# jdubkim/Self-play-on-Multi-Snakes-Environment

Hardware: AMD Instinct MI355X
Metric: env-steps/sec (agent·step) at 4 096×19×19×3-snake, 1/2/4/8 GPU + CPU ref (higher is better)
Workload: dtype u8

## Files before the change

### include/msnake.h

```cpp
#ifndef MSNAKE_H
#define MSNAKE_H

#include <stddef.h>
#include <stdint.h>

#ifdef __cplusplus
extern "C" {
#endif

#define MSNAKE_ABI_VERSION 3

#define MSNAKE_RULES_SNAKE_ENV 0
#define MSNAKE_RULES_NEW_WORLD 1
#define MSNAKE_RULES_ADVERSARIAL 2

#define MSNAKE_MAX_SNAKES 4
#define MSNAKE_MAX_FRUITS 32
#define MSNAKE_MAX_DIM 62

#define MSNAKE_OK 0
#define MSNAKE_E_ARG (-1)
#define MSNAKE_E_HIP (-2)
#define MSNAKE_E_HANDLE (-3)
#define MSNAKE_E_ALIGN (-4)
// ... 75 lines not shown
int msnake_set_state_all(msnake_handle h, const void* buf, size_t bytes);

typedef struct msnake_blob_info {
    int32_t version, num_envs, dim, n_snakes, n_fruits, rules;
    int64_t total_words;
} msnake_blob_info;
int msnake_state_blob_info(const void* buf, size_t bytes, msnake_blob_info* out);

int msnake_render(msnake_handle h, uint8_t* obs_dev, void* stream);

#define MSNAKE_POLICY_NONE 0
#define MSNAKE_POLICY_SAFE_GREEDY 1
#define MSNAKE_POLICY_HAMILTONIAN 2
int msnake_scripted_actions(msnake_handle h, int32_t policy, uint32_t snake_mask, int32_t* actions_dev,
                            int32_t action_stride, uint8_t* safe_dev, void* stream);

int msnake_space_actions(msnake_handle h, uint32_t snake_mask, int32_t* actions_dev, int32_t action_stride,
                         uint8_t* safe_dev, uint16_t* space_dev, void* stream);

int msnake_copy_envs(msnake_handle dst, msnake_handle src, const int32_t* src_index_dev, void* stream);

int msnake_render_cells(msnake_handle h, uint32_t view_mask, uint8_t* cells_dev, int32_t* snakes_dev, void* stream);

#define MSNAKE_LOCAL_MAX_RADIUS 31
#define MSNAKE_CELL_OUTSIDE 6
int msnake_render_local(msnake_handle h, int32_t radius, uint32_t snake_mask, int32_t oriented, uint8_t* windows_dev,
                        uint8_t* heading_dev, void* stream);

int msnake_get_stats(msnake_handle h, msnake_stats* out, int32_t reset);

const char* msnake_kernel_name(msnake_handle h);
int msnake_kernel_name_for_config(const msnake_config* cfg, char* out, size_t n);
int msnake_set_generic_kernels(int32_t on);
int64_t msnake_algorithmic_bytes_per_env_step(msnake_handle h);

#ifdef __cplusplus
}
#endif
#endif
```

### self-play-on-multi-snakes-environment_amd/_capi.py

```python
import ctypes
import os

_HERE = os.path.dirname(os.path.abspath(__file__))
LIB_PATH = os.environ.get("MSNAKE_LIB") or os.path.join(_HERE, "libmsnake.so")

RULES = {"snake_env": 0, "new_world": 1, "adversarial": 2}
RULE_NAMES = {v: k for k, v in RULES.items()}

SYMBOLS = [
    "msnake_abi_version", "msnake_last_error", "msnake_create", "msnake_destroy", "msnake_obs_shape",
    "msnake_reset", "msnake_reset_envs", "msnake_step", "msnake_step_tape", "msnake_rollout_tape", "msnake_get_state", "msnake_set_state",
    "msnake_get_state_all", "msnake_set_state_all", "msnake_state_blob_info",
    "msnake_render", "msnake_get_stats", "msnake_kernel_name", "msnake_algorithmic_bytes_per_env_step",
    "msnake_scripted_actions", "msnake_copy_envs", "msnake_kernel_name_for_config",
    "msnake_set_generic_kernels", "msnake_space_actions", "msnake_render_cells", "msnake_render_local",
]


class MsnakeConfig(ctypes.Structure):
    _fields_ = [("struct_size", ctypes.c_uint32), ("device", ctypes.c_int32), ("num_envs", ctypes.c_int32),
                ("dim", ctypes.c_int32), ("n_snakes", ctypes.c_int32), ("n_fruits", ctypes.c_int32),
                ("rules", ctypes.c_int32), ("max_steps", ctypes.c_int32), ("auto_reset", ctypes.c_int32),
                ("obs_scale", ctypes.c_int32), ("seed", ctypes.c_uint64), ("env_id_base", ctypes.c_uint64),
                ("envs_per_block", ctypes.c_int32), ("record_policy", ctypes.c_int32),
                ("obs_store_policy", ctypes.c_int32), ("tape_store_policy", ctypes.c_int32)]


ABI_VERSION = 3
CONFIG_SIZE_V2 = 56
RECORD_POLICY = {"auto": 0, "full": 1, "short": 2}
STORE_POLICY = {"auto": 0, "plain": 1, "stream": 2}
SCRIPTED_POLICY = {None: 0, "safe_greedy": 1, "hamiltonian": 2}
SPACE_POLICY = "space_greedy"


class MsnakeBlobInfo(ctypes.Structure):
    _fields_ = [("version", ctypes.c_int32), ("num_envs", ctypes.c_int32), ("dim", ctypes.c_int32),
                ("n_snakes", ctypes.c_int32), ("n_fruits", ctypes.c_int32), ("rules", ctypes.c_int32),
                ("total_words", ctypes.c_int64)]


class MsnakeStats(ctypes.Structure):
    _fields_ = [("episodes", ctypes.c_int64), ("ep_len_sum", ctypes.c_int64), ("ep_return_sum", ctypes.c_int64),
                ("env_steps", ctypes.c_int64), ("errors", ctypes.c_int64), ("reserved", ctypes.c_int64 * 3)]


_lib = None

# ... 10 lines not shown
            "(python -c 'import __graft_entry__ as g; g.build()' or make -C <pkg>/csrc). "
            "There is no CPU fallback.")
    import torch
    L = ctypes.CDLL(LIB_PATH)
    vp, i32, u8p = ctypes.c_void_p, ctypes.c_int32, ctypes.c_void_p
    L.msnake_abi_version.restype = ctypes.c_int
    L.msnake_last_error.restype = ctypes.c_char_p
    L.msnake_create.argtypes = [ctypes.POINTER(MsnakeConfig), ctypes.POINTER(vp)]
    L.msnake_destroy.argtypes = [vp]
    L.msnake_obs_shape.argtypes = [vp] + [ctypes.POINTER(i32)] * 3
    L.msnake_reset.argtypes = [vp, u8p, vp]
    L.msnake_render.argtypes = [vp, u8p, vp]
    L.msnake_reset_envs.argtypes = [vp, u8p, u8p, u8p, u8p, vp]
    L.msnake_step.argtypes = [vp, vp, i32, u8p, vp, vp, vp, vp]
    L.msnake_scripted_actions.argtypes = [vp, i32, ctypes.c_uint32, vp, i32, u8p, vp]
    L.msnake_space_actions.argtypes = [vp, ctypes.c_uint32, vp, i32, u8p, vp, vp]
    L.msnake_render_cells.argtypes = [vp, ctypes.c_uint32, u8p, vp, vp]
    L.msnake_render_local.argtypes = [vp, i32, ctypes.c_uint32, i32, u8p, u8p, vp]
    L.msnake_copy_envs.argtypes = [vp, vp, vp, vp]
    L.msnake_step_tape.argtypes = [vp, vp, i32, i32, u8p, ctypes.c_size_t, vp, vp, vp, ctypes.c_size_t, vp]
    L.msnake_rollout_tape.argtypes = L.msnake_step_tape.argtypes
    L.msnake_get_state.argtypes = [vp, i32, vp, i32]
    L.msnake_set_state.argtypes = [vp, i32, vp, i32]
    L.msnake_get_state_all.argtypes = [vp, vp, ctypes.c_size_t]
    L.msnake_get_state_all.restype = ctypes.c_int64
    L.msnake_set_state_all.argtypes = [vp, vp, ctypes.c_size_t]
    L.msnake_state_blob_info.argtypes = [vp, ctypes.c_size_t, ctypes.POINTER(MsnakeBlobInfo)]
    L.msnake_get_stats.argtypes = [vp, ctypes.POINTER(MsnakeStats), i32]
    L.msnake_kernel_name.argtypes = [vp]
    L.msnake_kernel_name.restype = ctypes.c_char_p
    L.msnake_kernel_name_for_config.argtypes = [ctypes.POINTER(MsnakeConfig), ctypes.c_char_p, ctypes.c_size_t]
    L.msnake_kernel_name_for_config.restype = ctypes.c_int
    L.msnake_set_generic_kernels.argtypes = [i32]
    L.msnake_set_generic_kernels.restype = ctypes.c_int
    L.msnake_algorithmic_bytes_per_env_step.argtypes = [vp]
    L.msnake_algorithmic_bytes_per_env_step.restype = ctypes.c_int64
    for name in ("msnake_create", "msnake_destroy", "msnake_obs_shape", "msnake_reset", "msnake_reset_envs", "msnake_render",
                 "msnake_step", "msnake_step_tape", "msnake_rollout_tape", "msnake_get_state", "msnake_set_state", "msnake_set_state_all",
                 "msnake_state_blob_info", "msnake_get_stats", "msnake_scripted_actions", "msnake_copy_envs",
                 "msnake_space_actions", "msnake_render_cells", "msnake_render_local"):
        getattr(L, name).restype = ctypes.c_int
    _lib = L
    return L


def apply_kernel_switch():
    load().msnake_set_generic_kernels(int(os.environ.get("MSNAKE_GENERIC_KERNELS", "") not in ("", "0")))


def kernel_name_for_config(cfg):
    apply_kernel_switch()
    buf = ctypes.create_string_buffer(64)
    check(load().msnake_kernel_name_for_config(ctypes.byref(cfg), buf, len(buf)), "msnake_kernel_name_for_config")
    return buf.value.decode()


def check(rc, what="msnake call"):
    if rc < 0:
        msg = load().msnake_last_error().decode("utf-8", "replace")
        raise RuntimeError(f"{what} failed ({rc}): {msg}")
    return rc
```

### self-play-on-multi-snakes-environment_amd/csrc/msnake_capi.hip

```cpp
#include <hip/hip_runtime.h>

#include <atomic>
#include <cstdarg>
#include <cstdio>
#include <cstdlib>
#include <cstring>
#include <vector>

#include "msnake_internal.h"

namespace {

thread_local char g_err[512] = "";

int fail(int code, const char* fmt, ...) {
    va_list ap;
    va_start(ap, fmt);
    vsnprintf(g_err, sizeof(g_err), fmt, ap);
    va_end(ap);
    return code;
}

#define HIP_TRY(expr)                                                                                   \
    do {                                                                                                \
// ... 617 lines not shown
    if (!out) return fail(MSNAKE_E_ARG, "msnake_get_stats: out is NULL");
    DeviceGuard guard(h->cfg.device);
    HIP_TRY(hipDeviceSynchronize());
    HIP_TRY(hipMemsetAsync(h->d_stats, 0, 64, nullptr));
    HIP_TRY(msnake::launch_stats(h->p.hdr, h->p.nenv, h->p.stats, reset ? 1 : 0, nullptr));
    unsigned long long raw[8];
    HIP_TRY(hipMemcpy(raw, h->d_stats, sizeof(raw), hipMemcpyDeviceToHost));
    memset(out, 0, sizeof(*out));
    out->episodes = (int64_t)raw[0];
    out->ep_len_sum = (int64_t)raw[1];
    out->ep_return_sum = (int64_t)raw[2];
    out->env_steps = h->env_steps;
    out->errors = (int64_t)raw[4];
    if (reset) h->env_steps = 0;
    return MSNAKE_OK;
}

const char* msnake_kernel_name(msnake_handle h) {
    if (check(h)) return "";
    return h->kname;
}

int msnake_kernel_name_for_config(const msnake_config* cfg_in, char* out, size_t n) {
    if (!cfg_in || !out || n == 0) return fail(MSNAKE_E_ARG, "msnake_kernel_name_for_config: NULL argument");
    msnake_config cfg;
    if (int rc = validate_config(cfg_in, &cfg)) return rc;
    msnake::StepParams p;
    memset(&p, 0, sizeof(p));
    if (int rc = derive_shape(&cfg, p)) return rc;
    msnake::step_kernel_name(cfg.rules, cfg.n_snakes, cfg.obs_scale, pick_spec_dim(p, cfg.rules), out, n);
    return MSNAKE_OK;
}

int msnake_set_generic_kernels(int32_t on) { return g_generic_kernels.exchange(on ? 1 : 0, std::memory_order_relaxed); }

int64_t msnake_algorithmic_bytes_per_env_step(msnake_handle h) {
    if (check(h)) return -1;
    const msnake::StepParams& p = h->p;
    return (int64_t)p.S * p.obs_scale * p.obs_scale + (int64_t)p.dim * p.dim + 4 * p.n_snakes + 5 + 16 * p.n_snakes + 16;
}

}
```

### self-play-on-multi-snakes-environment_amd/csrc/msnake_internal.h

```cpp
#ifndef MSNAKE_INTERNAL_H
#define MSNAKE_INTERNAL_H

#include <hip/hip_runtime.h>
#include <stdint.h>

#include "../../include/msnake.h"

#define MSNAKE_BLOCK_THREADS 512
#define MSNAKE_MAX_ENVS_PER_BLOCK 8

#define MSNAKE_HDR_WORDS 64
#define MSNAKE_HDR_SHORT_WORDS 32
#define SN_A(s) (0 + (s))
#define SN_B(s) (4 + (s))
#define SN_C(s) (8 + (s))
#define SN_C_HP0_SHIFT 24
#define HDR_T 12
#define HDR_CTR_LO 13
#define HDR_CTR_HI 14
#define HDR_FLAGS 15
#define HDR_FLAG_FINISHED 0x100u
#define HDR_EP_RETURN 16
#define HDR_EP_LEN 17
#define HDR_SPARE 18
// ... 51 lines not shown
    int32_t short_rec;
    int32_t stream_tape;
    int32_t spec_dim;
    uint8_t* state;
    uint32_t* hdr;
    uint16_t* body0;
    const uint8_t* tmpl;
    uint16_t* ring;
    uint16_t* fl0;
    uint16_t* flist;
    int32_t fcap;
    unsigned long long* stats;
    const int32_t* actions;
    uint8_t* obs;
    StepRest rest;
};

hipError_t launch_stats(uint32_t* hdr, int nenv, unsigned long long* stats, int clear, hipStream_t stream);
hipError_t launch_step(const StepParams& p, int rules, int mode, int envs_per_block, hipStream_t stream);
hipError_t launch_state_sizes(const StepParams& p, int rules, int env0, int count, uint32_t* need_words, hipStream_t stream);
hipError_t launch_state_pack(const StepParams& p, int rules, int env0, int count, const uint64_t* offsets, int32_t* words,
                             hipStream_t stream);
hipError_t launch_state_unpack(const StepParams& p, int rules, int env0, int count, const uint64_t* offsets,
                               const int32_t* words, uint32_t* status, hipStream_t stream);
hipError_t launch_scripted(const StepParams& p, int rules, int policy, uint32_t snake_mask, int32_t* actions, int32_t action_stride,
                           uint8_t* safe, hipStream_t stream);
hipError_t launch_space(const StepParams& p, int rules, uint32_t snake_mask, int32_t* actions, int32_t action_stride, uint8_t* safe,
                        uint16_t* space, hipStream_t stream);
hipError_t launch_copy_envs(const StepParams& dst, const StepParams& src, int rules, const int32_t* src_index, hipStream_t stream);
hipError_t launch_cells(const StepParams& p, int rules, uint32_t view_mask, uint8_t* cells, int32_t* snakes, hipStream_t stream);
hipError_t launch_local(const StepParams& p, int rules, int radius, uint32_t snake_mask, int oriented, uint8_t* windows,
                        uint8_t* heading, hipStream_t stream);
int spec_dim_of(const StepParams& p, int rules);
void step_kernel_name(int rules, int n_snakes, int obs_scale, int spec_dim, char* out, size_t n);

}

#endif
```

### self-play-on-multi-snakes-environment_amd/csrc/msnake_kernels.hip

```cpp
#include <hip/hip_runtime.h>
#include <stdint.h>
#include <stdio.h>
#include <stdlib.h>

#include <type_traits>

#include "msnake_internal.h"

namespace msnake {

__device__ __forceinline__ uint64_t ballot(bool p) { return __builtin_amdgcn_ballot_w64(p); }
__device__ __forceinline__ uint32_t rdlane(uint32_t v, int l) {
    return (uint32_t)__builtin_amdgcn_readlane((int)v, l);
}
__device__ __forceinline__ uint32_t uni(uint32_t v) { return (uint32_t)__builtin_amdgcn_readfirstlane((int)v); }
__device__ __forceinline__ void wave_sync() {
    __builtin_amdgcn_fence(__ATOMIC_RELEASE, "wavefront");
    __builtin_amdgcn_wave_barrier();
    __builtin_amdgcn_fence(__ATOMIC_ACQUIRE, "wavefront");
}
__device__ __forceinline__ uint32_t mbcnt(uint64_t m) {
    return __builtin_amdgcn_mbcnt_hi((uint32_t)(m >> 32), __builtin_amdgcn_mbcnt_lo((uint32_t)m, 0u));
}
template <int N>
// ... 99 lines not shown
    for (int b = 0; b < NB; ++b) w |= (uint64_t)pix_byte<J, VIEWS>(head, first + b) << (8 * b);
    return w;
}
typedef uint64_t __attribute__((aligned(1))) u64_unaligned;
typedef uint32_t __attribute__((aligned(1))) u32_unaligned;
typedef uint16_t __attribute__((aligned(1))) u16_unaligned;
template <int J, int VIEWS>
__device__ __forceinline__ void paint_pixel(uint8_t* p, bool head) {
    constexpr int C = 3 * VIEWS;
    if constexpr (C == 3) {
        constexpr uint16_t H = (uint16_t)pix_word<J, VIEWS, 2>(true, 0), B = (uint16_t)pix_word<J, VIEWS, 2>(false, 0);
        constexpr uint8_t H2 = pix_byte<J, VIEWS>(true, 2), B2 = pix_byte<J, VIEWS>(false, 2);
        *reinterpret_cast<u16_unaligned*>(p) = head ? H : B;
        p[2] = head ? H2 : B2;
    } else if constexpr (C == 6) {
        constexpr uint32_t H = (uint32_t)pix_word<J, VIEWS, 4>(true, 0), B = (uint32_t)pix_word<J, VIEWS, 4>(false, 0);
        constexpr uint16_t H4 = (uint16_t)pix_word<J, VIEWS, 2>(true, 4), B4 = (uint16_t)pix_word<J, VIEWS, 2>(false, 4);
        *reinterpret_cast<u32_unaligned*>(p) = head ? H : B;
        *reinterpret_cast<u16_unaligned*>(p + 4) = head ? H4 : B4;
    } else if constexpr (C == 9) {
        constexpr uint64_t H = pix_word<J, VIEWS, 8>(true, 0), B = pix_word<J, VIEWS, 8>(false, 0);
        constexpr uint8_t H8 = pix_byte<J, VIEWS>(true, 8), B8 = pix_byte<J, VIEWS>(false, 8);
        *reinterpret_cast<u64_unaligned*>(p) = head ? H : B;
        p[8] = head ? H8 : B8;
    } else {
        static_assert(C == 12, "views");
        constexpr uint64_t H = pix_word<J, VIEWS, 8>(true, 0), B = pix_word<J, VIEWS, 8>(false, 0);
        constexpr uint32_t H8 = (uint32_t)pix_word<J, VIEWS, 4>(true, 8), B8 = (uint32_t)pix_word<J, VIEWS, 4>(false, 8);
        *reinterpret_cast<u64_unaligned*>(p) = head ? H : B;
        *reinterpret_cast<u32_unaligned*>(p + 8) = head ? H8 : B8;
    }
}

template <int RULES, int NS, int MODE, int K, int DIM = 0>
__global__ __launch_bounds__(MSNAKE_BLOCK_THREADS) void msnake_step_kernel(
    uint8_t* __restrict__ state, uint8_t* __restrict__ obs, const int32_t* __restrict__ actions,
    float* __restrict__ rew_out, uint8_t* __restrict__ done_out, const int32_t nenv, const uint32_t pk0,
    const uint32_t pk1, const uint32_t pk2, const StepRest p) {
    constexpr int VIEWS = RULES == MSNAKE_RULES_NEW_WORLD ? NS : 3;
    constexpr int C = 3 * VIEWS;
    constexpr bool SPEC = DIM > 0;
    static_assert(!SPEC || (RULES == MSNAKE_RULES_SNAKE_ENV && K == 1 && (MODE == 0 || MODE == 3) && DIM <= MSNAKE_MAX_DIM),
                  "compile-time shapes: snake_env, native size, step / tape kernels");
    extern __shared__ __attribute__((aligned(16))) uint8_t smem[];
    int lane = (int)(threadIdx.x & 63u);
    const int wave = (int)uni(threadIdx.x >> 6);
    const uint32_t epb = (pk2 >> PK2_EPB_SHIFT) & 0xFFu;
    uint32_t b = blockIdx.x;
    b = (b & ~63u) | ((b & 7u) << 3) | ((b >> 3) & 7u);
    const int e = (int)(b * epb) + wave;
    if (e >= nenv) return;
    if ((MODE == 1 || MODE == 2) && p.env_mask && uni(p.env_mask[e]) == 0u) {
        if (MODE == 1 && p.truncated && lane == 0) p.truncated[e] = 0;
        return;
    }

    uint32_t pk0v = pk0, pk1v = pk1, pk2v = pk2;
    int dim, nf, action_stride, S, cap, W, n2, img_bytes, occ_bytes;
    bool auto_reset, short_rec;
    uint32_t max_steps;
    uint8_t *img, *bg;
    constexpr int FR0 = RULES == MSNAKE_RULES_NEW_WORLD ? HDR_FRUIT0_N : HDR_FRUIT0_S;
    constexpr bool LDSBG = MODE == 3 && K == 1;
    constexpr int TMPL_COPIES = K == 1 ? MSNAKE_TMPL_COPIES : 1;
#ifdef MSNAKE_NO_ALIGN
    constexpr bool CAN_ALIGN = false;
#else
    constexpr bool CAN_ALIGN = K == 1;
#endif
    const bool align_now = CAN_ALIGN && (MODE != 3 || (pk2 & PK2_TAPE_ALIGNED));
    auto unpack = [&]() {
        if constexpr (SPEC) {
            dim = DIM; nf = NS; action_stride = NS; auto_reset = true; short_rec = false;
            max_steps = pk0v >> 16;
            S = (DIM + 2) * (DIM + 2) * C; cap = (DIM * DIM + 2 + 63) / 64 * 64;
            W = DIM + 2; n2 = DIM * DIM;
// ... 349 lines not shown
        HV_SET_C(HDR_EP_RETURN, 0u);
        HV_SET_C(HDR_EP_LEN, 0u);
    }

    DBG_EXIT(1)
    const int n_steps = MODE == 3 ? p.n_steps : 1;
    float* rew_t = rew_out;
    uint8_t* done_t = done_out;
    msnake_info* info_t = p.info;
    uint8_t* obs_t = obs;
    uint32_t abatch = 0;
#pragma nounroll
    for (int step_i = 0; step_i < n_steps; ++step_i) {
    if (MODE == 3) {
        if (SPEC) asm volatile("" : "+v"(lane), "+s"(pk0v));
        else asm volatile("" : "+v"(lane), "+s"(pk0v), "+s"(pk1v), "+s"(pk2v));
        unpack();
        lds_layout();
        __builtin_amdgcn_s_setprio(0);
    }
    if (MODE == 3) {
        if (step_i > 0) {
            rew_t += p.scalar_step_stride; done_t += p.scalar_step_stride;
            if (info_t) info_t += p.scalar_step_stride;
            if (obs_t) obs_t += p.obs_step_stride;
        }
        if ((step_i & 15) == 0) {
            const int t = step_i + (lane >> 2);
            abatch = 0;
            if ((lane & 3) < NS && t < n_steps)
                abatch = (uint32_t)actions[((size_t)t * (size_t)nenv + (size_t)e) * action_stride + (lane & 3)];
        }
    }
    auto obs_shift_of = [&]() -> uint32_t {
        uint32_t ee = (uint32_t)e;
        if (FENCED) asm volatile("" : "+s"(ee));
        return (align_now && obs_t) ? (((uint32_t)(uintptr_t)obs_t + ee * (uint32_t)S) & 15u) : 0u;
    };
#ifdef MSNAKE_DBG_STAGES
    if (obs_t && (!LDSBG || step_i == 0) && !(dbg & 0x100)) {
#else
    if (obs_t && (!LDSBG || step_i == 0)) {
#endif
        const uint4* tsrc = reinterpret_cast<const uint4*>(tmpl_of() + (CAN_ALIGN ? obs_shift_of() * (uint32_t)img_bytes : 0u)) + lane;
        uint8_t* dst = LDSBG ? bg : img;
        const int nk = img_bytes >> 10;
#define MSNAKE_GP(k) ((const __attribute__((address_space(1))) void*)(tsrc + (k) * 64))
#define MSNAKE_LP(k) ((__attribute__((address_space(3))) void*)(dst + (k) * 1024))
        const uint32_t lds0 = (uint32_t)(uintptr_t)MSNAKE_LP(0);
        constexpr int NK_SPEC = SPEC ? ((DIM + 2) * (DIM + 2) * C + 15 + 1023) >> 10 : 0;
        if constexpr (NK_SPEC == 4)
            asm volatile("s_mov_b32 m0, %1\n\ts_nop 0\n\t"
                         "global_load_lds_dwordx4 %0, off\n\t"
                         "global_load_lds_dwordx4 %0, off offset:1024\n\t"
                         "global_load_lds_dwordx4 %0, off offset:2048\n\t"
                         "global_load_lds_dwordx4 %0, off offset:3072"
                         :: "v"(tsrc), "s"(uni(lds0)) : "m0", "memory");
        else if constexpr (NK_SPEC == 2)
            asm volatile("s_mov_b32 m0, %1\n\ts_nop 0\n\t"
                         "global_load_lds_dwordx4 %0, off\n\t"
                         "global_load_lds_dwordx4 %0, off offset:1024"
                         :: "v"(tsrc), "s"(uni(lds0)) : "m0", "memory");
        else
        asm volatile("s_mov_b32 m0, %1\n\ts_nop 0\n\t"
                     "global_load_lds_dwordx4 %0, off\n\t"
                     "s_cmp_lt_u32 %2, 2\n\ts_cbranch_scc1 1f\n\t"
                     "global_load_lds_dwordx4 %0, off offset:1024\n\t"
                     "s_cmp_lt_u32 %2, 3\n\ts_cbranch_scc1 1f\n\t"
                     "global_load_lds_dwordx4 %0, off offset:2048\n\t"
                     "s_cmp_lt_u32 %2, 4\n\ts_cbranch_scc1 1f\n\t"
                     "global_load_lds_dwordx4 %0, off offset:3072\n"
                     "1:"
                     :: "v"(tsrc), "s"(uni(lds0)), "s"(uni((uint32_t)nk)) : "m0", "scc", "memory");
        if (nk > 4)
            for (int k = 4; k < nk; ++k) __builtin_amdgcn_global_load_lds(MSNAKE_GP(k), MSNAKE_LP(k), 16, 0, 0);
#undef MSNAKE_GP
#undef MSNAKE_LP
    }
    uint32_t early = 0;
    uint32_t early_ok = 0;
    if (EARLY_PHILOX && !short_rec) {
        asm volatile("s_waitcnt lgkmcnt(0)" : "+s"(early_ctr), "+s"(early_pc));
        const uint32_t c_lo = (uint32_t)early_ctr, c_hi = (uint32_t)(early_ctr >> 32);
        const uint32_t pv = (uint32_t)early_pc, pb = (uint32_t)(early_pc >> 32);
        uint32_t used = (c_lo - pb) | ((pv ^ 1u) << 5);
        asm volatile("" : "+s"(used));
        if (used > (uint32_t)(HDR_PC_N - 4 * NS)) {
            early_ok = 1u;
            uint32_t ee = (uint32_t)e;
            asm volatile("" : "+s"(ee));
            const uint64_t gid = p.env_id_base + (uint64_t)ee;
            uint32_t k0 = p.seed_lo, k1 = p.seed_hi;
            asm volatile("" : "+s"(k0), "+s"(k1));
            const uint32_t b_lo = c_lo - (uint32_t)HDR_PC_FIRST, b_hi = c_hi - (c_lo < (uint32_t)HDR_PC_FIRST ? 1u : 0u);
            early = philox_draws(b_lo, b_hi, lane, (uint32_t)gid, (uint32_t)(gid >> 32), k0, k1);
            SPAN_FLAG(8u);
        }
    }
    if (!LDSBG || (step_i & 15) == 0) asm volatile("s_waitcnt vmcnt(0)" ::: "memory");
#if defined(MSNAKE_PAD_SALU) || defined(MSNAKE_PAD_VALU) || defined(MSNAKE_PAD_BRANCH)
    {
#ifdef MSNAKE_PAD_SALU
        uint32_t pad = pk0v;
#pragma unroll
        for (int i = 0; i < MSNAKE_PAD_SALU; ++i) asm volatile("s_add_u32 %0, %0, 1" : "+s"(pad) :: "scc");
        if (pad == 0xDEADBEEFu) hv = pad;
#endif
#ifdef MSNAKE_PAD_VALU
        uint32_t padv = (uint32_t)lane;
#pragma unroll
        for (int i = 0; i < MSNAKE_PAD_VALU; ++i) asm volatile("v_add_u32 %0, %0, 1" : "+v"(padv));
        if (padv == 0xDEADBEEFu) hv = padv;
#endif
#ifdef MSNAKE_PAD_BRANCH
#pragma unroll
        for (int i = 0; i < MSNAKE_PAD_BRANCH; ++i) asm volatile("s_cmp_eq_u32 0, 1\n\ts_cbranch_scc1 1f\n\ts_nop 0\n1:" ::: "scc");
#endif
    }
#endif
    asm volatile("" : "+s"(early_ok));
    if (EARLY_PHILOX && early_ok != 0) {
        hv = lane >= HDR_PC_FIRST ? early : hv;
        HV_SET_C(HDR_PC_BASE, (uint32_t)early_ctr);
        HV_SET_C(HDR_PC_VALID, 1u);
        upper_is_dirty();
    }
#pragma unroll
    for (int s = 0; s < NS; ++s) asm volatile("" : "+v"(cr[s]));
    if (MODE == 3) {
        const int a = __shfl((int)abatch, 4 * (step_i & 15) + lane);
// ... 398 lines not shown
        uint32_t out_len = 0;
        done = uni(done);
#ifdef MSNAKE_DBG_STAGES
        if (dbg & 0x1000) done = 0;
#endif
        asm volatile("" : "+s"(done));
#ifdef MSNAKE_LATE_REFILL
        slow_step = done | (any_eat ? 1u : 0u);
#endif
        if (done) {
            out_ret = ep_ret; out_len = ep_len;
            const uint32_t fl = rdlane(hv, HDR_FLAGS);
            if (!(fl & HDR_FLAG_FINISHED)) {
                if (lane == HDR_ACC_EPISODES) hv += 1u;
                if (lane == HDR_ACC_LEN) hv += ep_len;
                const bool carry = ballot(lane == HDR_ACC_LEN && hv < ep_len) != 0;
                if (carry && lane == HDR_ACC_LEN_HI) hv += 1u;
                if (lane == HDR_ACC_RETURN) hv += (uint32_t)(int)ep_ret;
                HV_SET_C(HDR_FLAGS, fl | HDR_FLAG_FINISHED);
            }
            if (auto_reset) {
                ep_ret = 0.0f; ep_len = 0;
                __builtin_amdgcn_s_setprio(3);
                do_reset();
            }
        }
        HV_SET_C(HDR_EP_RETURN, __float_as_uint(ep_ret));
        HV_SET_C(HDR_EP_LEN, ep_len);
        STAMP(4);
        DBG_EXIT(5)
        STAMP_FLAG((unsigned long long)(any_eat ? 1 : 0) | (done ? 2ull : 0ull));
        SPAN_FLAG((any_eat ? 1u : 0u) | (done ? 2u : 0u));
        SPAN(2);
        if (lane == 0) {
            rew_t[e] = reward;
            done_t[e] = (uint8_t)done;
            if (info_t) {
                int4 iv;
                iv.x = (int)__float_as_uint(out_ret); iv.y = (int)out_len; iv.z = num_alive; iv.w = (int)done;
                reinterpret_cast<int4*>(info_t)[e] = iv;
            }
        }
    }

    LANE_FENCE();
    CONFIG_FENCE();
    if (obs_t) {
#ifdef MSNAKE_PRIO_PAINT
        __builtin_amdgcn_s_setprio(MSNAKE_PRIO_PAINT);
#endif
        wave_sync();
        uint8_t* px = img + (CAN_ALIGN ? obs_shift_of() : 0u);
        if (RULES == MSNAKE_RULES_ADVERSARIAL) {
            for_each_fruit((int)rdlane(hv, HDR_NLIST), [&](int, uint32_t cell) {
                if (!in_grid(cell, dim)) return;
                const int off = ((int)(cell >> 8) * W + (int)(cell & 255u)) * (C * K);
#pragma unroll
                for (int k = 0; k < K; ++k)
#pragma unroll
                    for (int v = 0; v < VIEWS; ++v) px[off + k * C + 3 * v] = 255;
            });
        } else if (lane >= FR0 && lane < FR0 + nf) {
            const uint32_t cell = hv & 0xFFFFu;
            if (MODE != 2 || in_grid(cell, dim)) {
                const int off = ((int)(cell >> 8) * W + (int)(cell & 255u)) * (C * K);
#pragma unroll
                for (int k = 0; k < K; ++k)
#pragma unroll
                    for (int v = 0; v < VIEWS; ++v) px[off + k * C + 3 * v] = 255;
            }
        }
        const uint32_t flags = RULES == MSNAKE_RULES_NEW_WORLD ? rdlane(hv, HDR_FLAGS) : 0u;
#pragma unroll
        for (int j = 0; j < NS; ++j) {
            const uint32_t w0 = rdlane(hv, SN_A(j));
            if (RULES == MSNAKE_RULES_NEW_WORLD && !((flags >> j) & 1u)) continue;
            if (MODE == 2) pidx[j] = (lane - (int)(rdlane(hv, SN_C(j)) >> SN_C_HP0_SHIFT)) & 63;
            for_each_piece_at(j, cr[j], pidx[j], w0, (int)(w0 >> 16), [&](int i, uint32_t cell) {
                if ((MODE == 2 || !SPEC) && !in_grid(cell, dim)) return;
                const int off = ((int)(cell >> 8) * W + (int)(cell & 255u)) * (C * K);
#pragma unroll
                for (int k = 0; k < K; ++k) {
                    uint8_t* q = px + off + k * C;
                    if (j == 0) paint_pixel<0, VIEWS>(q, i == 0);
                    else if (j == 1) paint_pixel<1, VIEWS>(q, i == 0);
                    else if (j == 2) paint_pixel<2, VIEWS>(q, i == 0);
                    else paint_pixel<3, VIEWS>(q, i == 0);
                }
            });
        }
        wave_sync();
        STAMP(5);
        SPAN(3);
#ifdef MSNAKE_DBG_STAGES
        if (dbg == 6) asm volatile("s_endpgm");
#endif
#if defined(MSNAKE_PAD_SALU_COPYOUT)
        {
            uint32_t pad = pk0v;
#pragma unroll
            for (int i = 0; i < MSNAKE_PAD_SALU_COPYOUT; ++i) asm volatile("s_add_u32 %0, %0, 1" : "+s"(pad) :: "scc");
            if (pad == 0xDEADBEEFu) hv = pad;
        }
#endif
        if (align_now) {
            uint8_t* obs_env = obs_t + (size_t)e * S;
            const uint32_t obs_shift = obs_shift_of();
            uint8_t* g_al = obs_env - obs_shift;
            const int lead = (int)(((uint32_t)(uintptr_t)g_al >> 4) & 7u);
            const int end = (int)obs_shift + DBG_NO_OBS_STORES(S);
            const int kmin = (int)((obs_shift + 15u) >> 4);
            const uint32_t nk = (uint32_t)((end >> 4) - kmin);
            const int k0 = lane - lead;
            const uint32_t rel = (uint32_t)(k0 - kmin);
            const uint8_t* lsrc = img + 16 * k0;
            uint8_t* gdst = g_al + 16 * k0;
            auto chunks = [&](auto NT) {
#pragma unroll
                for (int i = 0; i < 4; ++i) {
                    if (rel + 64u * i < nk DBG_FEWER_STORES(i)) {
                        const u32x4 v = *reinterpret_cast<const u32x4*>(lsrc + 1024 * i);
                        if constexpr (decltype(NT)::value) __builtin_nontemporal_store(v, reinterpret_cast<u32x4*>(gdst + 1024 * i));
                        else *reinterpret_cast<u32x4*>(gdst + 1024 * i) = v;
                        if constexpr (SPEC) {
                            if constexpr (decltype(NT)::value) asm volatile("; streaming copy-out" ::: "memory");
                            else asm volatile("; plain copy-out" ::: "memory");
                        }
                    }
                }
                if ((!SPEC || ((S + 15) >> 4) + 7 > 256) && nk + (uint32_t)(kmin + lead) > 256u)
                    for (uint32_t r = rel + 256u; r < nk; r += 64u) {
                        const u32x4 v = *reinterpret_cast<const u32x4*>(lsrc + 16 * (r - rel));
                        if constexpr (decltype(NT)::value) __builtin_nontemporal_store(v, reinterpret_cast<u32x4*>(gdst + 16 * (size_t)(r - rel)));
                        else *reinterpret_cast<u32x4*>(gdst + 16 * (size_t)(r - rel)) = v;
                    }
            };
            if (pk2 & (MODE == 3 ? PK2_STREAM_TAPE : PK2_STREAM_OBS)) chunks(std::true_type{});
            else chunks(std::false_type{});
// ... 62 lines not shown
#ifdef MSNAKE_LATE_REFILL
        if (PCACHE && !short_rec && MODE != 3) {
            const uint32_t ctr_lo = rdlane(hv, HDR_CTR_LO);
            bool late;
            if (refilled != 0)
                late = !(draws_n == 64 && ctr_lo - draw_base + HDR_PC_N <= 64u);
            else if (MSNAKE_LATE_REFILL == 0)
                late = rdlane(hv, HDR_PC_VALID) != 1u || ctr_lo - rdlane(hv, HDR_PC_BASE) > HDR_PC_N - 5u * NS;
            else
                late = slow_step == 0 && (rdlane(hv, HDR_PC_VALID) != 1u || ctr_lo - rdlane(hv, HDR_PC_BASE) >= (uint32_t)(MSNAKE_LATE_REFILL));
            if (late) {
                SPAN_FLAG(8u);
                refill_draws(ctr_lo, rdlane(hv, HDR_CTR_HI));
            }
        }
#endif
        if (PCACHE && (!NUMFLAGS ? (refilled != 0 && !short_rec) : uni(refilled) == 1u)) {
            upper_is_dirty();
            const uint32_t ctr_lo = rdlane(hv, HDR_CTR_LO);
            const uint32_t off = ctr_lo - draw_base;
            if (draws_n == 64 && off + HDR_PC_N <= 64u) {
                const uint32_t sh = (uint32_t)__shfl((int)draws, lane - HDR_PC_FIRST + (int)off);
                hv = lane >= HDR_PC_FIRST ? sh : hv;
                HV_SET_C(HDR_PC_BASE, ctr_lo);
                HV_SET_C(HDR_PC_VALID, 1u);
            } else {
                HV_SET_C(HDR_PC_VALID, 0u);
            }
        }
        const uint32_t rec_words = uni((uint32_t)MSNAKE_HDR_SHORT_WORDS + ((!NUMFLAGS && short_rec) ? 0u : rec_extra));
        if ((uint32_t)lane < rec_words) {
            uint32_t ee = (uint32_t)e;
            if (MODE == 3) asm volatile("" : "+s"(ee));
            (reinterpret_cast<uint32_t*>(state) + (size_t)ee * MSNAKE_HDR_WORDS)[lane] = hv;
        }
        if (RULES == MSNAKE_RULES_ADVERSARIAL && fr_dirty) fl0_of()[lane] = (uint16_t)fr;
    }
#ifdef MSNAKE_END_WAIT
    asm volatile("s_waitcnt vmcnt(0)" ::: "memory");
#endif
#ifdef MSNAKE_HAVE_SPAN
    if (p.dbg_span) {
        SPAN(4);
        asm volatile("s_waitcnt vmcnt(0)" ::: "memory");
        SPAN(5);
        uint32_t xcc;
        asm volatile("s_getreg_b32 %0, hwreg(HW_REG_XCC_ID)" : "=s"(xcc));
        if (lane == 0) p.dbg_span[(size_t)e * 8 + 6] = dbgf | ((xcc & 15u) << 8);
    }
#endif
}

__global__ __launch_bounds__(256) void msnake_stats_kernel(uint32_t* __restrict__ hdr, int nenv,
                                                           unsigned long long* __restrict__ stats, int clear) {
    long long ep = 0, ln = 0, rt = 0, er = 0;
    for (int e = (int)(blockIdx.x * blockDim.x + threadIdx.x); e < nenv; e += (int)(gridDim.x * blockDim.x)) {
        uint32_t* h = hdr + (size_t)e * MSNAKE_HDR_WORDS;
        ep += h[HDR_ACC_EPISODES]; ln += (long long)(((unsigned long long)h[HDR_ACC_LEN_HI] << 32) | h[HDR_ACC_LEN]);
        rt += (int)h[HDR_ACC_RETURN]; er += h[HDR_ACC_ERRORS];
        if (clear) h[HDR_ACC_EPISODES] = h[HDR_ACC_LEN] = h[HDR_ACC_LEN_HI] = h[HDR_ACC_RETURN] = h[HDR_ACC_ERRORS] = 0u;
    }
#pragma unroll
    for (int o = 32; o > 0; o >>= 1) {
        ep += __shfl_down(ep, o); ln += __shfl_down(ln, o); rt += __shfl_down(rt, o); er += __shfl_down(er, o);
    }
    if ((threadIdx.x & 63u) == 0) {
        atomicAdd(&stats[0], (unsigned long long)ep);
// ... 188 lines not shown
                       state_view(p, rules), env0, count, offsets, words);
    return hipGetLastError();
}

hipError_t launch_state_unpack(const StepParams& p, int rules, int env0, int count, const uint64_t* offsets,
                               const int32_t* words, uint32_t* status, hipStream_t stream) {
    hipLaunchKernelGGL(msnake_state_unpack_kernel, dim3((unsigned)((count + 3) / 4)), dim3(256), 0, stream,
                       state_view(p, rules), env0, count, offsets, words, status);
    return hipGetLastError();
}

static uint32_t div_magic(uint32_t dim) {
    uint32_t bits = 0;
    while ((dim >> bits) != 0) ++bits;
    return (uint32_t)((1ull << (14u + bits)) / dim) + 1u;
}

static constexpr bool has_spec(int rules, int ns, int k, int dim) {
    return rules == MSNAKE_RULES_SNAKE_ENV && k == 1 && ((dim == 19 && (ns == 2 || ns == 3)) || (dim == 10 && ns == 1));
}
int spec_dim_of(const StepParams& p, int rules) {
    if (!has_spec(rules, p.n_snakes, p.obs_scale, p.dim)) return 0;
    const int W = p.dim + 2, n2 = p.dim * p.dim, S = W * W * 9;
    if (p.n_fruits != p.n_snakes || !p.auto_reset || p.short_rec || p.views != 3 || p.C != 9) return 0;
    if (p.S != S || p.rest.cap != (n2 + 2 + 63) / 64 * 64 || p.img_bytes != ((S + 15 + 1023) & ~1023) ||
        p.lds_per_wave != p.img_bytes + ((n2 + 15) & ~15))
        return 0;
    return p.dim;
}
static int spec_dim_now(const StepParams& p, int mode) {
    return (p.spec_dim != 0 && (mode == 0 || mode == 3) && p.action_stride == p.n_snakes) ? p.spec_dim : 0;
}

template <int RULES, int NS, int K>
static hipError_t launch_k(const StepParams& p, int mode, int epb, hipStream_t stream) {
    const uint32_t pk0 = (uint32_t)p.dim | ((uint32_t)p.n_fruits << 6) | ((uint32_t)p.action_stride << 12) |
                         ((uint32_t)(p.auto_reset ? 1 : 0) << 15) | ((uint32_t)p.rest.max_steps << 16);
    const uint32_t pk1 = (uint32_t)p.S | ((uint32_t)p.rest.cap << 16);

    size_t lds_wave = (size_t)p.lds_per_wave;
    if (mode == 3 && K == 1) {
        lds_wave += (size_t)p.img_bytes;
        while (epb > 1 && lds_wave * (size_t)epb > 64 * 1024) epb >>= 1;
        if (lds_wave > 64 * 1024) return hipErrorInvalidValue;
    }
    const size_t lds = lds_wave * (size_t)epb;
    bool nt_obs = p.rest.stream_obs != 0;
    if (K > 1) {
        const size_t OB = (size_t)p.S * K * K;
        nt_obs = nt_obs && mode != 3 && p.obs && OB % 16 == 0 && ((uintptr_t)p.obs & 15) == 0 && OB < (1u << 24);
    }
    const uint32_t pk2 = (p.short_rec ? PK2_SHORT_REC : 0u) | (nt_obs ? PK2_STREAM_OBS : 0u) |
                         (p.stream_tape && K == 1 ? PK2_STREAM_TAPE : 0u) |
                         (mode == 3 && K == 1 && p.rest.obs_step_stride % 16 == 0 ? PK2_TAPE_ALIGNED : 0u) | ((uint32_t)epb << PK2_EPB_SHIFT) |
                         (div_magic((uint32_t)p.dim) << PK2_DIVM_SHIFT);
    const dim3 grid((unsigned)((((p.nenv + epb - 1) / epb) + 63) & ~63));
    const dim3 block(64u * (unsigned)epb);
#define MSNAKE_LAUNCH_D(M, D)                                                                                     \
    hipLaunchKernelGGL((msnake_step_kernel<RULES, NS, M, K, D>), grid, block, lds, stream, p.state, p.obs, p.actions, \
                       p.rest.rew, p.rest.done, p.nenv, pk0, pk1, pk2, p.rest)
#define MSNAKE_LAUNCH(M) MSNAKE_LAUNCH_D(M, 0)
    constexpr int SPEC_DIM = has_spec(RULES, NS, K, 19) ? 19 : has_spec(RULES, NS, K, 10) ? 10 : 0;
    if constexpr (SPEC_DIM != 0) {
        if (spec_dim_now(p, mode) == SPEC_DIM) {
            if (mode == 0) MSNAKE_LAUNCH_D(0, SPEC_DIM);
            else MSNAKE_LAUNCH_D(3, SPEC_DIM);
            return hipGetLastError();
        }
    }
    switch (mode) {
        case 0: MSNAKE_LAUNCH(0); break;
        case 1: MSNAKE_LAUNCH(1); break;
        case 3: MSNAKE_LAUNCH(3); break;
        default: MSNAKE_LAUNCH(2); break;
    }
#undef MSNAKE_LAUNCH
#undef MSNAKE_LAUNCH_D
    return hipGetLastError();
}

template <int RULES, int NS>
static hipError_t launch_ns(const StepParams& p, int mode, int epb, hipStream_t stream) {
    switch (p.obs_scale) {
        case 1: return launch_k<RULES, NS, 1>(p, mode, epb, stream);
        case 4: return launch_k<RULES, NS, 4>(p, mode, epb, stream);
        case 7: return launch_k<RULES, NS, 7>(p, mode, epb, stream);
        default: return hipErrorInvalidValue;
    }
}

template <int RULES>
static hipError_t launch_rules(const StepParams& p, int mode, int epb, hipStream_t stream) {
    switch (p.n_snakes) {
        case 1: return launch_ns<RULES, 1>(p, mode, epb, stream);
        case 2: return launch_ns<RULES, 2>(p, mode, epb, stream);
        case 3: return launch_ns<RULES, 3>(p, mode, epb, stream);
        case 4:
            if (RULES == MSNAKE_RULES_NEW_WORLD) return launch_ns<MSNAKE_RULES_NEW_WORLD, 4>(p, mode, epb, stream);
            return hipErrorInvalidValue;
        default: return hipErrorInvalidValue;
    }
}

hipError_t launch_step(const StepParams& p, int rules, int mode, int epb, hipStream_t stream) {
    if (epb < 1 || epb > MSNAKE_MAX_ENVS_PER_BLOCK) return hipErrorInvalidValue;
    switch (rules) {
        case MSNAKE_RULES_SNAKE_ENV: return launch_rules<MSNAKE_RULES_SNAKE_ENV>(p, mode, epb, stream);
        case MSNAKE_RULES_NEW_WORLD: return launch_rules<MSNAKE_RULES_NEW_WORLD>(p, mode, epb, stream);
        case MSNAKE_RULES_ADVERSARIAL: return launch_rules<MSNAKE_RULES_ADVERSARIAL>(p, mode, epb, stream);
        default: return hipErrorInvalidValue;
// ... 16 lines not shown
```

Baseline: 777.8 million.

## Add plain-call step kernel variant with precomputed copy-out geometry and folded null checks

Adds a PLAIN template variant of the compile-time-shape step kernel. The host selects it when obs, rew, done and info are all non-null, obs is 128-byte aligned and offsets fit in 32 bits. The variant drops the runtime null-pointer branches and uses 32-bit offset arithmetic for the scalar and header stores. It also precomputes per-lane store masks for the aligned obs copy-out, using compile-time classification of which 1 KiB chunks are always, partially or never active. The aim is to cut scalar/vector overhead and branching in the per-step obs write-out. The cost is another kernel instantiation, more code complexity, and a new API for querying the call shape.

Measured after the change: 797.6 million, median of 6. +2.5%, better.

```diff
diff --git a/include/msnake.h b/include/msnake.h
--- a/include/msnake.h
+++ b/include/msnake.h
@@ -131,6 +131,11 @@
 const char* msnake_kernel_name(msnake_handle h);
 int msnake_kernel_name_for_config(const msnake_config* cfg, char* out, size_t n);
 int msnake_set_generic_kernels(int32_t on);
+#define MSNAKE_CALL_GENERIC 0
+#define MSNAKE_CALL_SHAPE 1
+#define MSNAKE_CALL_PLAIN 2
+int msnake_call_shape_for_config(const msnake_config* cfg, int32_t action_stride, const void* obs_dev, const void* rew_dev,
+                                 const void* done_dev, const void* info_dev, int32_t* out);
 int64_t msnake_algorithmic_bytes_per_env_step(msnake_handle h);
 
 #ifdef __cplusplus
diff --git a/self-play-on-multi-snakes-environment_amd/_capi.py b/self-play-on-multi-snakes-environment_amd/_capi.py
--- a/self-play-on-multi-snakes-environment_amd/_capi.py
+++ b/self-play-on-multi-snakes-environment_amd/_capi.py
@@ -14,6 +14,7 @@
     "msnake_render", "msnake_get_stats", "msnake_kernel_name", "msnake_algorithmic_bytes_per_env_step",
     "msnake_scripted_actions", "msnake_copy_envs", "msnake_kernel_name_for_config",
     "msnake_set_generic_kernels", "msnake_space_actions", "msnake_render_cells", "msnake_render_local",
+    "msnake_call_shape_for_config",
 ]
 
 
@@ -90,6 +91,8 @@
     L.msnake_kernel_name_for_config.argtypes = [ctypes.POINTER(MsnakeConfig), ctypes.c_char_p, ctypes.c_size_t]
     L.msnake_kernel_name_for_config.restype = ctypes.c_int
     L.msnake_set_generic_kernels.argtypes = [i32]
+    L.msnake_call_shape_for_config.argtypes = [ctypes.POINTER(MsnakeConfig), i32, vp, vp, vp, vp, ctypes.POINTER(i32)]
+    L.msnake_call_shape_for_config.restype = ctypes.c_int
     L.msnake_set_generic_kernels.restype = ctypes.c_int
     L.msnake_algorithmic_bytes_per_env_step.argtypes = [vp]
     L.msnake_algorithmic_bytes_per_env_step.restype = ctypes.c_int64
@@ -113,6 +116,17 @@
     return buf.value.decode()
 
 
+CALL_SHAPE = {0: "generic", 1: "shape", 2: "plain"}
+
+
+def call_shape_for_config(cfg, action_stride, obs, rew, done, info):
+    apply_kernel_switch()
+    out = ctypes.c_int32(-1)
+    check(load().msnake_call_shape_for_config(ctypes.byref(cfg), action_stride, obs or None, rew or None, done or None,
+                                              info or None, ctypes.byref(out)), "msnake_call_shape_for_config")
+    return CALL_SHAPE[out.value]
+
+
 def check(rc, what="msnake call"):
     if rc < 0:
         msg = load().msnake_last_error().decode("utf-8", "replace")
diff --git a/self-play-on-multi-snakes-environment_amd/csrc/msnake_capi.hip b/self-play-on-multi-snakes-environment_amd/csrc/msnake_capi.hip
--- a/self-play-on-multi-snakes-environment_amd/csrc/msnake_capi.hip
+++ b/self-play-on-multi-snakes-environment_amd/csrc/msnake_capi.hip
@@ -673,6 +673,26 @@
     return MSNAKE_OK;
 }
 
+int msnake_call_shape_for_config(const msnake_config* cfg_in, int32_t action_stride, const void* obs_dev, const void* rew_dev,
+                                 const void* done_dev, const void* info_dev, int32_t* out) {
+    if (!cfg_in || !out) return fail(MSNAKE_E_ARG, "msnake_call_shape_for_config: NULL argument");
+    msnake_config cfg;
+    if (int rc = validate_config(cfg_in, &cfg)) return rc;
+    msnake::StepParams p;
+    memset(&p, 0, sizeof(p));
+    if (int rc = derive_shape(&cfg, p)) return rc;
+    if (action_stride < p.n_snakes || action_stride > 7)
+        return fail(MSNAKE_E_ARG, "action_stride %d must be in [n_snakes=%d, 7]", action_stride, p.n_snakes);
+    p.spec_dim = pick_spec_dim(p, cfg.rules);
+    p.action_stride = action_stride;
+    p.obs = static_cast<uint8_t*>(const_cast<void*>(obs_dev));
+    p.rest.rew = static_cast<float*>(const_cast<void*>(rew_dev));
+    p.rest.done = static_cast<uint8_t*>(const_cast<void*>(done_dev));
+    p.rest.info = static_cast<msnake_info*>(const_cast<void*>(info_dev));
+    *out = msnake::call_shape_of(p, 0);
+    return MSNAKE_OK;
+}
+
 int msnake_set_generic_kernels(int32_t on) { return g_generic_kernels.exchange(on ? 1 : 0, std::memory_order_relaxed); }
 
 int64_t msnake_algorithmic_bytes_per_env_step(msnake_handle h) {
diff --git a/self-play-on-multi-snakes-environment_amd/csrc/msnake_internal.h b/self-play-on-multi-snakes-environment_amd/csrc/msnake_internal.h
--- a/self-play-on-multi-snakes-environment_amd/csrc/msnake_internal.h
+++ b/self-play-on-multi-snakes-environment_amd/csrc/msnake_internal.h
@@ -107,6 +107,7 @@
 hipError_t launch_local(const StepParams& p, int rules, int radius, uint32_t snake_mask, int oriented, uint8_t* windows,
                         uint8_t* heading, hipStream_t stream);
 int spec_dim_of(const StepParams& p, int rules);
+int call_shape_of(const StepParams& p, int mode);
 void step_kernel_name(int rules, int n_snakes, int obs_scale, int spec_dim, char* out, size_t n);
 
 }
diff --git a/self-play-on-multi-snakes-environment_amd/csrc/msnake_kernels.hip b/self-play-on-multi-snakes-environment_amd/csrc/msnake_kernels.hip
--- a/self-play-on-multi-snakes-environment_amd/csrc/msnake_kernels.hip
+++ b/self-play-on-multi-snakes-environment_amd/csrc/msnake_kernels.hip
@@ -155,7 +155,31 @@
     }
 }
 
-template <int RULES, int NS, int MODE, int K, int DIM = 0>
+enum { PG_NEVER = 0, PG_PARTIAL = 1, PG_ALWAYS = 2 };
+template <int S_>
+struct PlainGeom {
+    static constexpr int S = S_;
+    static constexpr int kind(int i) {
+        bool any = false, all = true;
+        for (int shift = 0; shift < 16; ++shift) {
+            const int kmin = shift != 0 ? 1 : 0, nk = ((shift + S) >> 4) - kmin;
+            for (int lead = 0; lead < 8; ++lead) {
+                const int lo = 64 * i - lead - kmin, hi = lo + 63;
+                const bool lo_on = lo >= 0 && lo < nk, hi_on = hi >= 0 && hi < nk;
+                any = any || lo_on || hi_on || (lo < 0 && hi >= nk && nk > 0);
+                all = all && lo_on && hi_on;
+            }
+        }
+        return all ? PG_ALWAYS : any ? PG_PARTIAL : PG_NEVER;
+    }
+    uint64_t m[4];
+    uint64_t edge;
+    uint32_t gal;
+    uint32_t k0off;
+    uint32_t tail;
+};
+
+template <int RULES, int NS, int MODE, int K, int DIM = 0, int PLAIN = 0>
 __global__ __launch_bounds__(MSNAKE_BLOCK_THREADS) void msnake_step_kernel(
     uint8_t* __restrict__ state, uint8_t* __restrict__ obs, const int32_t* __restrict__ actions,
     float* __restrict__ rew_out, uint8_t* __restrict__ done_out, const int32_t nenv, const uint32_t pk0,
@@ -165,6 +189,9 @@
     constexpr bool SPEC = DIM > 0;
     static_assert(!SPEC || (RULES == MSNAKE_RULES_SNAKE_ENV && K == 1 && (MODE == 0 || MODE == 3) && DIM <= MSNAKE_MAX_DIM),
                   "compile-time shapes: snake_env, native size, step / tape kernels");
+    static_assert(PLAIN == 0 || (SPEC && MODE == 0), "plain calls: the per-step kernels of the compile-time shapes");
+    constexpr bool FOLD = PLAIN != 0;
+    constexpr bool EGEOM = PLAIN != 0;
     extern __shared__ __attribute__((aligned(16))) uint8_t smem[];
     int lane = (int)(threadIdx.x & 63u);
     const int wave = (int)uni(threadIdx.x >> 6);
@@ -580,15 +607,18 @@
                 abatch = (uint32_t)actions[((size_t)t * (size_t)nenv + (size_t)e) * action_stride + (lane & 3)];
         }
     }
+    const uint32_t pc_eo = EGEOM ? (uint32_t)e * (uint32_t)S : 0u;
+    const uint32_t pc_shift = pc_eo & 15u;
     auto obs_shift_of = [&]() -> uint32_t {
+        if constexpr (EGEOM) return pc_shift;
         uint32_t ee = (uint32_t)e;
         if (FENCED) asm volatile("" : "+s"(ee));
-        return (align_now && obs_t) ? (((uint32_t)(uintptr_t)obs_t + ee * (uint32_t)S) & 15u) : 0u;
+        return (align_now && (FOLD || obs_t)) ? (((uint32_t)(uintptr_t)obs_t + ee * (uint32_t)S) & 15u) : 0u;
     };
 #ifdef MSNAKE_DBG_STAGES
-    if (obs_t && (!LDSBG || step_i == 0) && !(dbg & 0x100)) {
+    if ((FOLD || obs_t) && (!LDSBG || step_i == 0) && !(dbg & 0x100)) {
 #else
-    if (obs_t && (!LDSBG || step_i == 0)) {
+    if ((FOLD || obs_t) && (!LDSBG || step_i == 0)) {
 #endif
         const uint4* tsrc = reinterpret_cast<const uint4*>(tmpl_of() + (CAN_ALIGN ? obs_shift_of() * (uint32_t)img_bytes : 0u)) + lane;
         uint8_t* dst = LDSBG ? bg : img;
@@ -644,6 +674,36 @@
             early = philox_draws(b_lo, b_hi, lane, (uint32_t)gid, (uint32_t)(gid >> 32), k0, k1);
             SPAN_FLAG(8u);
         }
+    }
+    using PG = PlainGeom<(DIM + 2) * (DIM + 2) * C>;
+    PG pg = {};
+    auto plain_geom = [&]() {
+        if constexpr (EGEOM) {
+            const uint32_t lead = (pc_eo >> 4) & 7u;
+            const uint32_t kmin = (pc_shift + 15u) >> 4;
+            const uint32_t end = pc_shift + (uint32_t)PG::S;
+            const uint32_t nk = (end >> 4) - kmin;
+            const uint32_t rel = (uint32_t)lane - lead - kmin;
+            if constexpr (PG::kind(0) == PG_PARTIAL) pg.m[0] = ballot(rel < nk);
+            if constexpr (PG::kind(1) == PG_PARTIAL) pg.m[1] = ballot(rel + 64u < nk);
+            if constexpr (PG::kind(2) == PG_PARTIAL) pg.m[2] = ballot(rel + 128u < nk);
+            if constexpr (PG::kind(3) == PG_PARTIAL) pg.m[3] = ballot(rel + 192u < nk);
+            pg.gal = pc_eo - pc_shift;
+            pg.k0off = 0u - 16u * lead;
+            pg.tail = (end & ~15u) - 16u;
+            const bool head = lane < 16;
+            const uint32_t first = head ? pc_shift : 16u;
+            const uint32_t count = head ? ((16u - pc_shift) & 15u) : (end & 15u);
+            pg.edge = ballot((uint32_t)lane - first < count);
+        }
+    };
+    if constexpr (EGEOM) {
+        plain_geom();
+        if constexpr (PG::kind(0) == PG_PARTIAL) asm volatile("" : "+s"(pg.m[0]));
+        if constexpr (PG::kind(1) == PG_PARTIAL) asm volatile("" : "+s"(pg.m[1]));
+        if constexpr (PG::kind(2) == PG_PARTIAL) asm volatile("" : "+s"(pg.m[2]));
+        if constexpr (PG::kind(3) == PG_PARTIAL) asm volatile("" : "+s"(pg.m[3]));
+        asm volatile("" : "+s"(pg.edge), "+s"(pg.gal), "+s"(pg.k0off), "+s"(pg.tail));
     }
     if (!LDSBG || (step_i & 15) == 0) asm volatile("s_waitcnt vmcnt(0)" ::: "memory");
 #if defined(MSNAKE_PAD_SALU) || defined(MSNAKE_PAD_VALU) || defined(MSNAKE_PAD_BRANCH)
@@ -1108,7 +1168,17 @@
         STAMP_FLAG((unsigned long long)(any_eat ? 1 : 0) | (done ? 2ull : 0ull));
         SPAN_FLAG((any_eat ? 1u : 0u) | (done ? 2u : 0u));
         SPAN(2);
-        if (lane == 0) {
+        if (FOLD) {
+            if (lane == 0) {
+                uint32_t ev = (uint32_t)e;
+                asm volatile("" : "+v"(ev));
+                *reinterpret_cast<float*>(reinterpret_cast<uint8_t*>(rew_t) + (size_t)(ev * 4u)) = reward;
+                done_t[(size_t)ev] = (uint8_t)done;
+                int4 iv;
+                iv.x = (int)__float_as_uint(out_ret); iv.y = (int)out_len; iv.z = num_alive; iv.w = (int)done;
+                *reinterpret_cast<int4*>(reinterpret_cast<uint8_t*>(info_t) + (size_t)(ev * 16u)) = iv;
+            }
+        } else if (lane == 0) {
             rew_t[e] = reward;
             done_t[e] = (uint8_t)done;
             if (info_t) {
@@ -1121,7 +1191,7 @@
 
     LANE_FENCE();
     CONFIG_FENCE();
-    if (obs_t) {
+    if (FOLD || obs_t) {
 #ifdef MSNAKE_PRIO_PAINT
         __builtin_amdgcn_s_setprio(MSNAKE_PRIO_PAINT);
 #endif
@@ -1179,7 +1249,34 @@
             if (pad == 0xDEADBEEFu) hv = pad;
         }
 #endif
-        if (align_now) {
+        if constexpr (EGEOM) {
+            const uint32_t k0b = ((uint32_t)lane << 4) + pg.k0off;
+            const uint8_t* lsrc = img + (int32_t)k0b;
+            uint8_t* gdst = obs_t + (size_t)(pg.gal + k0b);
+            auto chunks = [&](auto NT) {
+                auto one = [&](auto I) {
+                    constexpr int i = decltype(I)::value;
+                    if constexpr (PG::kind(i) != PG_NEVER) {
+                        if (PG::kind(i) == PG_ALWAYS || in_mask(pg.m[i])) {
+                            const u32x4 v = *reinterpret_cast<const u32x4*>(lsrc + 1024 * i);
+                            if constexpr (decltype(NT)::value) __builtin_nontemporal_store(v, reinterpret_cast<u32x4*>(gdst + 1024 * i));
+                            else *reinterpret_cast<u32x4*>(gdst + 1024 * i) = v;
+                            if constexpr (decltype(NT)::value) asm volatile("; streaming copy-out" ::: "memory");
+                            else asm volatile("; plain copy-out" ::: "memory");
+                        }
+                    }
+                };
+                one(std::integral_constant<int, 0>{}); one(std::integral_constant<int, 1>{});
+                one(std::integral_constant<int, 2>{}); one(std::integral_constant<int, 3>{});
+            };
+            static_assert(!EGEOM || ((PG::S + 15) >> 4) + 7 <= 256, "plain calls: the image fits the four store instructions");
+            if (pk2 & PK2_STREAM_OBS) chunks(std::true_type{});
+            else chunks(std::false_type{});
+            if (in_mask(pg.edge)) {
+                const uint32_t byte = lane < 16 ? (uint32_t)lane : pg.tail + (uint32_t)lane;
+                obs_t[(size_t)(pg.gal + byte)] = img[byte];
+            }
+        } else if (align_now) {
             uint8_t* obs_env = obs_t + (size_t)e * S;
             const uint32_t obs_shift = obs_shift_of();
             uint8_t* g_al = obs_env - obs_shift;
@@ -1308,7 +1405,9 @@
         if ((uint32_t)lane < rec_words) {
             uint32_t ee = (uint32_t)e;
             if (MODE == 3) asm volatile("" : "+s"(ee));
-            (reinterpret_cast<uint32_t*>(state) + (size_t)ee * MSNAKE_HDR_WORDS)[lane] = hv;
+            if (FOLD)
+                *reinterpret_cast<uint32_t*>(state + (size_t)(ee * (uint32_t)(MSNAKE_HDR_WORDS * 4) + (uint32_t)lane * 4u)) = hv;
+            else (reinterpret_cast<uint32_t*>(state) + (size_t)ee * MSNAKE_HDR_WORDS)[lane] = hv;
         }
         if (RULES == MSNAKE_RULES_ADVERSARIAL && fr_dirty) fl0_of()[lane] = (uint16_t)fr;
     }
@@ -1563,6 +1662,19 @@
     return (p.spec_dim != 0 && (mode == 0 || mode == 3) && p.action_stride == p.n_snakes) ? p.spec_dim : 0;
 }
 
+int call_shape_of(const StepParams& p, int mode) {
+    if (spec_dim_now(p, mode) == 0) return MSNAKE_CALL_GENERIC;
+    if (mode != 0) return MSNAKE_CALL_SHAPE;
+    const bool plain = p.obs && p.rest.info && p.rest.rew && p.rest.done && ((uintptr_t)p.obs & 127u) == 0 &&
+                       (uint64_t)p.nenv * (uint64_t)p.S < (1ull << 31);
+    return plain ? MSNAKE_CALL_PLAIN : MSNAKE_CALL_SHAPE;
+}
+#if defined(MSNAKE_DBG_STAGES) || defined(MSNAKE_NO_ALIGN)
+static constexpr bool PLAIN_BUILT = false;
+#else
+static constexpr bool PLAIN_BUILT = true;
+#endif
+
 template <int RULES, int NS, int K>
 static hipError_t launch_k(const StepParams& p, int mode, int epb, hipStream_t stream) {
     const uint32_t pk0 = (uint32_t)p.dim | ((uint32_t)p.n_fruits << 6) | ((uint32_t)p.action_stride << 12) |
@@ -1587,15 +1699,17 @@
                          (div_magic((uint32_t)p.dim) << PK2_DIVM_SHIFT);
     const dim3 grid((unsigned)((((p.nenv + epb - 1) / epb) + 63) & ~63));
     const dim3 block(64u * (unsigned)epb);
-#define MSNAKE_LAUNCH_D(M, D)                                                                                     \
-    hipLaunchKernelGGL((msnake_step_kernel<RULES, NS, M, K, D>), grid, block, lds, stream, p.state, p.obs, p.actions, \
+#define MSNAKE_LAUNCH_DP(M, D, P)                                                                                    \
+    hipLaunchKernelGGL((msnake_step_kernel<RULES, NS, M, K, D, P>), grid, block, lds, stream, p.state, p.obs, p.actions, \
                        p.rest.rew, p.rest.done, p.nenv, pk0, pk1, pk2, p.rest)
+#define MSNAKE_LAUNCH_D(M, D) MSNAKE_LAUNCH_DP(M, D, 0)
 #define MSNAKE_LAUNCH(M) MSNAKE_LAUNCH_D(M, 0)
     constexpr int SPEC_DIM = has_spec(RULES, NS, K, 19) ? 19 : has_spec(RULES, NS, K, 10) ? 10 : 0;
     if constexpr (SPEC_DIM != 0) {
         if (spec_dim_now(p, mode) == SPEC_DIM) {
-            if (mode == 0) MSNAKE_LAUNCH_D(0, SPEC_DIM);
-            else MSNAKE_LAUNCH_D(3, SPEC_DIM);
+            if (mode == 3) MSNAKE_LAUNCH_D(3, SPEC_DIM);
+            else if (PLAIN_BUILT && call_shape_of(p, mode) == MSNAKE_CALL_PLAIN) MSNAKE_LAUNCH_DP(0, SPEC_DIM, 1);
+            else MSNAKE_LAUNCH_D(0, SPEC_DIM);
             return hipGetLastError();
         }
     }
@@ -1607,6 +1721,7 @@
     }
 #undef MSNAKE_LAUNCH
 #undef MSNAKE_LAUNCH_D
+#undef MSNAKE_LAUNCH_DP
     return hipGetLastError();
 }
 
```
